# supersimple33/aruco-slam

Hardware: AMD Instinct MI355X
Metric: EKF updates/sec at n=1024 landmarks, m=32 obs/frame (higher is better)
Workload: dtype f32 covariance / f64 state

## Files before the change

aruco_slam_amd/csrc/ekf_api.hip:

```cpp
#include <atomic>
#include <cstring>

#include "ekf_host.h"
#include "ekf_kernels.h"

thread_local std::string g_err;

namespace {

std::atomic<ekf_filter*> g_pipelining{nullptr};

void release_pipelining_token(ekf_filter* f) { (void)g_pipelining.compare_exchange_strong(f, nullptr); }

constexpr int kStageSlots = 64;
constexpr int kMacroSuper = 8;
constexpr int kMacroMinTiles = 3000;
constexpr int kTimedKernels = 4;
constexpr int kWideVisible = 1024;
inline int visible_cap(int model) { return model == EKF_MODEL_ROTATIONS ? 50 : 64; }
inline bool wide_frame(int model, int m) { return m > visible_cap(model); }
constexpr int kEventPool = 2048;

struct Layout {
    int64_t cap;
// ... 197 lines not shown
    fr.jac = f->at<double>(L.off_jac);
    fr.resid = f->at<double>(L.off_resid);
    fr.lmcol = f->at<int32_t>(L.off_lmcol);
    fr.amat = f->at<double>(L.off_amat);
    fr.lda = L.cap;
    fr.sblk = f->at<double>(L.off_sblk);
    fr.sblk_rows = L.kmax;
    fr.lmat = f->at<double>(L.off_lmat);
    fr.ldl = L.kmax;
    fr.dinv = f->at<double>(L.off_dinv);
    fr.lop = f->at<double>(L.off_lop);
    fr.dop = f->at<double>(L.off_dop);
    fr.yvec = f->at<double>(L.off_y);
    fr.wpanel = f->at<void>(L.off_wpanel);
    fr.ldw = L.cap;
    fr.wdbg = f->debug_w ? f->at<double>(L.off_wdbg) : nullptr;
    fr.status = f->at<int32_t>(L.off_status);
    fr.traj_row = traj_row;
    fr.dxvec = f->at<double>(L.off_dx);
    fr.stamps = (f->debug_w || f->debug_stamps) ? f->at<long long>(L.off_stamps) : nullptr;
    fr.stamps_heavy = f->debug_stamps_light ? 0 : 1;
    fr.nz = EkfNoise{f->cfg.q_cam, f->cfg.q_err, f->cfg.q_lm, f->cfg.r_uncertainty};
    fr.quat_mode = f->cfg.quat_mode;
    fr.n_lm = f->n_lm;
    fr.state_host = nullptr;
    fr.status_host = nullptr;
    fr.cov_tiles = nullptr;
    fr.cov_grid = 0;
    if (f->tiles_T > 0 && f->tiles_T == (fr.dims + 127) / 128) {
        fr.cov_tiles = f->at<uint32_t>(L.off_tiles);
        fr.cov_grid = f->tiles_grid;
    }
    return fr;
}

bool use_front_kernel(const ekf_filter* f, const EkfFrame& fr) { return (f->cfg.flags & 4) == 0 && fr.kpad <= 192; }

void bind_exchange(ekf_filter* f, EkfFrame& fr) {
    const Layout& L = f->lay;
    double* base = f->at<double>(L.off_xl);
    fr.xl = base + (f->fseq & 1) * L.xl_len;
    fr.xl_next = base + ((f->fseq + 1) & 1) * L.xl_len;
    fr.xl_dop = (int32_t)L.xl_dop;
    fr.xl_y = (int32_t)L.xl_y;
    fr.xl_jac = (int32_t)L.xl_jac;
    fr.xl_tag = (int32_t)L.xl_tag;
    fr.xl_len = (int32_t)L.xl_len;
    fr.xs = fr.xl + L.xl_xs;
    fr.xr = fr.xl + L.xl_xr;
    fr.xs_tag = fr.xl + L.xl_stag;
    fr.seqno = (double)(f->fseq + 1);
    fr.done_ctr = f->at<unsigned long long>(L.off_done);
    f->done_total += (uint64_t)(fr.ncols / 64);
    fr.done_target = f->done_total;
    f->fseq++;
}

int ensure_tiles(ekf_filter* f) {
    const Layout& L = f->lay;
    const int T = (f->dims() + 127) / 128;
    const bool want = L.tiles_cap > 0 &&
                      (f->cfg.cov_kernel == EKF_COVK_MFMA_MACRO || T * (T + 1) / 2 >= kMacroMinTiles);
    if (!want) {
        f->tiles_T = -1;
        return EKF_OK;
    }
    if (f->tiles_T == T) return EKF_OK;
    HIP_TRY(hipStreamSynchronize(f->stream));
    HIP_TRY(hipStreamSynchronize(f->big));
    const int grid = ekf_cov_macro_table(T, kMacroSuper, f->tiles_host.at<uint32_t>(0), L.tiles_cap);
    if (grid <= 0) return fail(EKF_ERR_STATE, "macro-tile launch table does not fit the workspace");
    HIP_TRY(hipMemcpy(f->at<uint32_t>(L.off_tiles), f->tiles_host.get(), (size_t)grid * 4, hipMemcpyHostToDevice));
    f->tiles_T = T;
    f->tiles_grid = grid;
    return EKF_OK;
}

int enqueue_frame(ekf_filter* f, const int32_t* idx_dev, const double* z_dev, int m,
                  double* traj_row, bool mirror) {
    int trc = ensure_tiles(f);
    if (trc) return trc;
    EkfFrame fr = make_frame(f, idx_dev, z_dev, m, traj_row);
    const int variant = f->cfg.cov_kernel == EKF_COVK_VALU ? 1 : 2;
    hipEvent_t* ev = nullptr;
    if (f->timing) {
        if (f->ev_frames == kEventPool) {
            int rc = fold_timing(f);
            if (rc) return rc;
        }
        ev = &f->ev[f->ev_frames * (kTimedKernels + 1)];
        f->ev_frames++;
    }
    hipEvent_t* ev_all = (ev && !f->timing_cov_only) ? ev : nullptr;
    if (ev_all) HIP_TRY(hipEventRecord(ev[0], f->stream));
    const bool mirrored = use_front_kernel(f, fr) && !f->timing && mirror;
    if (use_front_kernel(f, fr)) {
        bind_exchange(f, fr);
        if (mirrored) {
            fr.state_host = f->readback.at<double>(256);
            fr.status_host = f->readback.at<int32_t>(128);
        }
        by_cov_type(f, [&](auto elem) { ekf_launch_front<decltype(elem)>(fr, f->stream); });
        if (ev_all) {
            HIP_TRY(hipEventRecord(ev[1], f->stream));
            HIP_TRY(hipEventRecord(ev[2], f->stream));
        }
    } else if (wide_frame(fr.model, m)) {
        const bool blocked = fr.kpad > EKF_WIDE_REUSE_ROWS;
        const int rp = blocked ? (int)round_up(fr.k, EKF_WIDE_BLOCK) : fr.kpad;
        double* aw = blocked ? f->at<double>(f->lay.off_wwork) : nullptr;
        if (blocked && !f->lay.off_wwork) return fail(EKF_ERR_STATE, "internal: no wide-frame workspace");
        by_cov_type(f, [&](auto elem) { ekf_launch_wide_front<decltype(elem)>(fr, aw, rp, f->stream); });
        if (ev_all) HIP_TRY(hipEventRecord(ev[1], f->stream));
        if (blocked) ekf_launch_wide_factor(fr, aw, f->at<double>(f->lay.off_xinv), rp, f->stream);
        else ekf_launch_solve(fr, f->stream);
        if (ev_all) HIP_TRY(hipEventRecord(ev[2], f->stream));
        by_cov_type(f, [&](auto elem) {
            if (blocked) ekf_launch_wide_finish<decltype(elem)>(fr, aw, f->stream);
            else ekf_launch_panel<decltype(elem)>(fr, f->stream);
        });
        if (fr.model == 1) ekf_launch_inject_rot(fr, f->n_lm, f->stream);
    } else {
        by_cov_type(f, [&](auto elem) { ekf_launch_gather<decltype(elem)>(fr, f->stream); });
        if (ev_all) HIP_TRY(hipEventRecord(ev[1], f->stream));
        ekf_launch_solve(fr, f->stream);
        if (ev_all) HIP_TRY(hipEventRecord(ev[2], f->stream));
        by_cov_type(f, [&](auto elem) { ekf_launch_panel<decltype(elem)>(fr, f->stream); });
        if (fr.model == 1) ekf_launch_inject_rot(fr, f->n_lm, f->stream);
    }
    f->shortcut.frame(!f->timing && hipEventRecord(f->ev_front, f->stream) == hipSuccess, mirrored);
    if (fr.kpad > EKF_WIDE_REUSE_ROWS) {
        if (ev) HIP_TRY(hipEventRecord(ev[3], f->stream));
        for (int r0 = 0; r0 < fr.kpad; r0 += EKF_WIDE_REUSE_ROWS) {
            EkfFrame cf = fr;
            cf.wpanel = static_cast<char*>(fr.wpanel) + (size_t)r0 * fr.ldw * f->lay.elem;
            cf.kpad = std::min(EKF_WIDE_REUSE_ROWS, fr.kpad - r0);
            cf.k = std::min(cf.kpad, std::max(0, fr.k - r0));
            if (r0 > 0) cf.nz.q_cam = cf.nz.q_err = cf.nz.q_lm = 0.0;
            by_cov_type(f, [&](auto elem) { ekf_launch_cov_update<decltype(elem)>(cf, variant, f->stream); });
        }
        if (ev) HIP_TRY(hipEventRecord(ev[4], f->stream));
    } else {
        by_cov_type(f, [&](auto elem) {
            ekf_launch_cov_update<decltype(elem)>(fr, variant, f->stream, ev ? ev[3] : nullptr, ev ? ev[4] : nullptr);
        });
    }
    HIP_TRY(hipGetLastError());
    f->last_m = m;
    return EKF_OK;
}

int check_ready(ekf_filter* f) {
    if (!f) return fail(EKF_ERR_INVALID, "filter handle is NULL");
    if (!f->bound) return fail(EKF_ERR_STATE, "ekf_bind_buffers has not been called");
    if (!f->is_reset) return fail(EKF_ERR_STATE, "ekf_reset has not been called");
    HIP_TRY(hipSetDevice(f->device));
    return EKF_OK;
}

int sync_and_check(ekf_filter* f, int state_count = 0) {
    if (state_count > 0 && f->shortcut.front_pending) {
        HIP_TRY(hipEventSynchronize(f->ev_front));
        if (f->shortcut.zero_copy() && *f->readback.at<volatile int32_t>(128) == 0)
            return EKF_OK;
        HIP_TRY(hipMemcpyAsync(f->readback.get(), f->at<int32_t>(f->lay.off_status), 32, hipMemcpyDeviceToHost, f->big));
        HIP_TRY(hipMemcpyAsync(f->readback.at<double>(256), f->state, (size_t)state_count * 8, hipMemcpyDeviceToHost, f->big));
        HIP_TRY(hipStreamSynchronize(f->big));
    } else {
        HIP_TRY(hipMemcpyAsync(f->readback.get(), f->at<int32_t>(f->lay.off_status), 32, hipMemcpyDeviceToHost, f->stream));
        if (state_count > 0)
            HIP_TRY(hipMemcpyAsync(f->readback.at<double>(256), f->state, (size_t)state_count * 8, hipMemcpyDeviceToHost, f->stream));
        HIP_TRY(hipStreamSynchronize(f->stream));
        release_pipelining_token(f);
    }
    const int32_t* info = f->readback.at<int32_t>(0);
    const int32_t st = info[0];
    f->shortcut.read_back(st == 0, state_count == f->dims());
    if (st != 0) {
        if (st & EKF_ST_BAD_INDEX)
            return fail(EKF_ERR_INVALID, "landmark index out of range in a device-resident detection array "
                                         "(clamped on the device; the filter state is no longer meaningful, reset it)");
        if (st & (EKF_ST_STALE_JAC | EKF_ST_STALE_COL | EKF_ST_STALE_S))
            return fail(EKF_ERR_NUMERIC, "internal: exchange data of another frame accepted in the front kernel (status " +
                                             std::to_string(st) + ")");
        if (st & EKF_ST_GATE_TIMEOUT)
            return fail(EKF_ERR_NUMERIC, "internal: a device-side wait between the two streams of the pipelined sequence mode timed out");
        if (st & EKF_ST_TIMEOUT)
            return fail(EKF_ERR_NUMERIC, "internal: exchange wait timed out in the front kernel (status " +
                                             std::to_string(st) + ")");
        if (info[2] >= 200)
            return fail(EKF_ERR_NUMERIC, "internal: a wait inside the factorisation workgroup timed out (flag word " +
                                             std::to_string(info[2] - 200) + ")");
        return fail(EKF_ERR_NUMERIC, "innovation covariance S was not positive definite (block column " +
                                         std::to_string(info[2] - 100) + ", wave mask " + std::to_string(info[1]) + ")");
    }
    return EKF_OK;
}

bool pipeline_wanted(const ekf_filter* f, int dims, int kpad, int m) {
    const bool auto_on = !(dims > 9000 && kpad > 96) && !(f->cfg.model == EKF_MODEL_ROTATIONS && kpad > 64);
    const bool want = (f->cfg.flags & 2) != 0 || ((f->cfg.flags & 1) == 0 && auto_on);
    return want && f->lay.has_cov2 && !f->timing && (f->cfg.flags & 4) == 0 && kpad <= 192 &&
           !wide_frame(f->cfg.model, m);
}

int probe_queues(ekf_filter* f) {
    if (f->la_ok >= 0) return EKF_OK;
    unsigned long long* probe = f->at<unsigned long long>(f->lay.off_sync) + 2;
    int32_t* pstat = f->at<int32_t>(f->lay.off_sync) + 8;
    f->la_ok = 0;
    for (int attempt = 0; attempt < 8 && f->la_ok == 0; ++attempt) {
        if (attempt > 0) {
            hipStream_t fresh = nullptr;
            HIP_TRY(hipStreamCreateWithFlags(&fresh, hipStreamNonBlocking));
            HIP_TRY(hipStreamSynchronize(f->big));
            (void)hipStreamDestroy(f->big);
            f->big = fresh;
        }
        HIP_TRY(hipMemsetAsync(probe, 0, 64, f->stream));
        HIP_TRY(hipStreamSynchronize(f->stream));
        ekf_launch_gate(probe, 1ull, pstat, f->big, 1 << 14);
        ekf_launch_signal(probe, 1ull, f->stream);
        HIP_TRY(hipStreamSynchronize(f->big));
        HIP_TRY(hipStreamSynchronize(f->stream));
        int32_t ps = 0;
        HIP_TRY(hipMemcpy(&ps, pstat, 4, hipMemcpyDeviceToHost));
        f->la_ok = (ps == 0) ? 1 : 0;
    }
    return EKF_OK;
}

bool take_pipelining_token(ekf_filter* f) {
    ekf_filter* owner = nullptr;
    if (!g_pipelining.compare_exchange_strong(owner, f) && owner != f) {
        bool idle = hipStreamQuery(owner->stream) == hipSuccess && hipStreamQuery(owner->big) == hipSuccess;
        (void)hipGetLastError();
        if (!(idle && g_pipelining.compare_exchange_strong(owner, f))) return false;
    }
    return true;
}

int choose_pipelining(ekf_filter* f, bool want_runs, int* mode) {
    *mode = EKF_SEQ_SERIAL;
    if (!want_runs) return EKF_OK;
    int rc = probe_queues(f);
    if (rc) return rc;
    if (f->la_ok == 0) *mode = EKF_SEQ_SERIAL_ONE_QUEUE;
    else if (!take_pipelining_token(f)) *mode = EKF_SEQ_SERIAL_OTHER_HANDLE;
    else *mode = EKF_SEQ_PIPELINED;
    return EKF_OK;
}

struct RunFrame {
    const int32_t* idx;
    const double* z;
    int m;
    double* traj_row;
};

template <class FrameAt>
int run_pipelined(ekf_filter* f, int frames, FrameAt frame_at, void* other) {
    const Layout& L = f->lay;
    int rc = ensure_tiles(f);
    if (rc) return rc;
    void* wbuf[2] = {f->at<void>(L.off_wpanel), f->at<void>(L.off_wpanel2)};
    void* cbuf[2] = {f->cov, other};
    char* wsup0 = f->at<char>(L.off_wsup);
    void* wsup[2] = {wsup0, wsup0 + (size_t)L.kmax * L.wsup_ld * L.elem};
    unsigned long long* sync = f->at<unsigned long long>(L.off_sync);
    int32_t* status = f->at<int32_t>(L.off_status);
    const uint64_t base = f->la_base;
    f->shortcut.run();
    RunFrame nx = frame_at(0);
    for (int t = 0; t < frames; ++t) {
        const int par = t & 1;
        const RunFrame cf_t = nx;
        EkfFrame fr = make_frame(f, cf_t.idx, cf_t.z, cf_t.m, cf_t.traj_row);
        fr.cov = cbuf[0];
        fr.wpanel = wbuf[par];
        if (t > 0) {
            fr.cov = cbuf[par ^ 1];
            fr.wprev = wbuf[par ^ 1];
            fr.wsup_prev = wsup[par ^ 1];
        }
        const int nb = fr.kpad / EKF_RB;
        const int grid = nb * (nb + 1) / 2 + 2 + fr.ncols / 64;
        fr.wsup_ld = L.wsup_ld;
        fr.la_sync = sync;
        fr.la_signal = (t > 0) ? base + (uint64_t)t : 0;
        fr.la_gate = (t > 0) ? base + (uint64_t)t : 0;
        fr.lds_min = grid <= 100 ? 148 * 1024 : 0;
        if (t + 1 < frames) {
            nx = frame_at(t + 1);
            fr.next_idx = nx.idx;
            fr.next_m = nx.m;
            fr.wsup = wsup[par];
        }
        bind_exchange(f, fr);
        by_cov_type(f, [&](auto elem) { ekf_launch_front<decltype(elem)>(fr, f->stream); });
        EkfFrame cu = fr;
        cu.cov = cbuf[par];
        cu.cov_out = cbuf[par ^ 1];
        if (t + 1 < frames) {
            ekf_launch_gate(sync, base + (uint64_t)t + 1, status, f->big);
            by_cov_type(f, [&](auto elem) { ekf_launch_cov_update<decltype(elem)>(cu, 2, f->big); });
            ekf_launch_signal(sync + 1, base + (uint64_t)t + 1, f->big);
        } else {
            by_cov_type(f, [&](auto elem) { ekf_launch_cov_update<decltype(elem)>(cu, 2, f->stream); });
        }
        HIP_TRY(hipGetLastError());
        f->last_m = cf_t.m;
    }
    f->cov = cbuf[frames & 1];
    f->la_base = base + (uint64_t)frames;
    return EKF_OK;
}

struct RunPlan {
    std::vector<char> candidate;
    std::vector<char> joins;
    bool want_runs = false;
};

template <class MOf, class NNewOf>
RunPlan plan_runs(const ekf_filter* f, int frames, MOf m_of, NNewOf nnew_of) {
    RunPlan p;
    p.candidate.assign((size_t)frames, 0);
    p.joins.assign((size_t)frames, 0);
    int prev_kpad = -1;
    int nn = f->n_lm;
    for (int t = 0; t < frames; ++t) {
        const int m = m_of(t);
        if (m == 0) continue;
        const int nnew = nnew_of(t);
        nn += nnew;
        const int kpad = (int)round_up(f->lay.rd * m, EKF_RB);
        p.candidate[t] = pipeline_wanted(f, f->lay.lmd * nn + EKF_CAM, kpad, m);
        p.joins[t] = p.candidate[t] && nnew == 0 && prev_kpad == kpad;
        p.want_runs = p.want_runs || p.joins[t];
        prev_kpad = p.candidate[t] ? kpad : -1;
    }
    return p;
}

template <class FrameOf, class FirstSightings>
int run_frames(ekf_filter* f, int frames, FrameOf frame_of, FirstSightings first_sightings, const RunPlan& plan, bool pipe_ok,
               int64_t* stats) {
    void* const home = f->cov;
    void* const spare = f->lay.has_cov2 ? f->at<void>(f->lay.off_cov2) : nullptr;
    std::vector<int> run;
    auto serial = [&](int t) {
        const RunFrame r = frame_of(t);
        if (stats) stats[0] += 1;
        return enqueue_frame(f, r.idx, r.z, r.m, r.traj_row, false);
    };
    auto flush = [&]() -> int {
        int rc = EKF_OK;
        if (run.size() == 1) {
            rc = serial(run[0]);
        } else if (run.size() >= 2) {
            rc = run_pipelined(f, (int)run.size(), [&](int i) { return frame_of(run[i]); }, f->cov == home ? spare : home);
            if (stats) {
                stats[0] += (int64_t)run.size();
                stats[1] += (int64_t)run.size();
                stats[2] += 1;
            }
        }
        run.clear();
        return rc;
    };
    int rc = EKF_OK;
    for (int t = 0; t < frames && rc == EKF_OK; ++t) {
        if (frame_of(t).m == 0) continue;
        const bool in_run = pipe_ok && plan.candidate[t];
        if (!(in_run && plan.joins[t])) {
            rc = flush();
            if (rc) break;
        }
        const int nnew = first_sightings(t);
        f->n_lm += nnew;
        if (stats) stats[3] += nnew;
        if (in_run) run.push_back(t);
        else rc = serial(t);
    }
    if (rc == EKF_OK) rc = flush();
    if (f->cov != home) {
        hipError_t e = hipMemcpyAsync(home, f->cov, (size_t)f->lay.cap * f->lay.cap * f->lay.elem, hipMemcpyDeviceToDevice,
                                      f->stream);
        f->cov = home;
        if (e != hipSuccess && rc == EKF_OK) rc = fail(EKF_ERR_HIP, std::string("hipMemcpyAsync: ") + hipGetErrorString(e));
    }
    return rc;
}

int reserve_host_buffers(ekf_filter* f, const Layout& L) {
    int rc = f->ring.reserve(L.slot_bytes * kStageSlots);
    if (rc == EKF_OK) rc = f->tiles_host.reserve((size_t)L.tiles_cap * 4);
    if (rc == EKF_OK) rc = f->readback.reserve(256 + (size_t)L.cap * 8);
    return rc;
}

int open_handle(ekf_filter* f) {
    int rc = reserve_host_buffers(f, f->lay);
    if (rc) return rc;
    HIP_TRY(hipStreamCreateWithFlags(&f->big, hipStreamNonBlocking));
    HIP_TRY(hipEventCreateWithFlags(&f->ev_front, hipEventDisableTiming));
    for (hipEvent_t& e : f->slot_done) HIP_TRY(hipEventCreateWithFlags(&e, hipEventDisableTiming));
    return EKF_OK;
}

int clear_buffers(const ekf_filter* f, void* cov, double* state, char* ws, const Layout& L) {
    HIP_TRY(hipMemsetAsync(cov, 0, (size_t)L.cap * L.cap * L.elem, f->stream));
    HIP_TRY(hipMemsetAsync(state, 0, (size_t)L.cap * 8, f->stream));
    HIP_TRY(hipMemsetAsync(ws, 0, L.total, f->stream));
    HIP_TRY(hipMemsetD32Async(reinterpret_cast<hipDeviceptr_t>(ws + L.off_xl), (int)0xFFFBADC0u, L.xl_len * 4, f->stream));
    return EKF_OK;
}

void restart_workspace(ekf_filter* f) {
    f->fseq = 0;
    f->done_total = 0;
    f->la_base = 0;
    f->tiles_T = -1;
    std::memset(f->readback.get(), 0, 256 + (size_t)f->lay.cap * 8);
}

}

extern "C" {

const char* ekf_last_error_string(void) { return g_err.c_str(); }

int ekf_default_config(ekf_config* cfg) {
    if (!cfg) return fail(EKF_ERR_INVALID, "config is NULL");
    std::memset(cfg, 0, sizeof(*cfg));
    cfg->max_landmarks = 50;
    cfg->max_visible = 50;
    cfg->cov_dtype = EKF_COV_F64;
    cfg->quat_mode = EKF_QUAT_AS_WRITTEN;
    cfg->cov_kernel = EKF_COVK_AUTO;
    cfg->model = EKF_MODEL_EKF;
    cfg->initial_camera_uncertainty = 0.1;
    cfg->initial_landmark_uncertainty = 0.7;
    cfg->r_uncertainty = 0.9;
    cfg->q_cam = 0.3;
    cfg->q_err = 0.5;
    cfg->q_lm = 0.01;
    cfg->stream = nullptr;
    return EKF_OK;
}

int ekf_query_sizes(const ekf_config* cfg, int64_t* ld, size_t* cov_bytes, size_t* state_bytes,
                    size_t* workspace_bytes) {
    int rc = check_config(cfg);
    if (rc) return rc;
    Layout L = make_layout(*cfg);
    if (ld) *ld = L.cap;
    if (cov_bytes) *cov_bytes = (size_t)L.cap * L.cap * L.elem;
    if (state_bytes) *state_bytes = (size_t)L.cap * 8;
    if (workspace_bytes) *workspace_bytes = L.total;
    return EKF_OK;
}

int ekf_create(const ekf_config* cfg, ekf_filter** out) {
    int rc = check_config(cfg);
    if (rc) return rc;
    if (!out) return fail(EKF_ERR_INVALID, "out is NULL");
    int ndev = 0;
    HIP_TRY(hipGetDeviceCount(&ndev));
    if (ndev < 1) return fail(EKF_ERR_HIP, "no HIP device visible");
    ekf_filter* f = new ekf_filter();
    if (hipGetDevice(&f->device) != hipSuccess) f->device = 0;
    f->cfg = *cfg;
    f->lay = make_layout(*cfg);
    f->stream = static_cast<hipStream_t>(cfg->stream);
    rc = open_handle(f);
    if (rc) {
        ekf_destroy(f);
        return rc;
    }
    *out = f;
    return EKF_OK;
}

int ekf_destroy(ekf_filter* f) {
    if (!f) return EKF_OK;
    (void)hipStreamSynchronize(f->stream);
    if (f->big) {
        (void)hipStreamSynchronize(f->big);
        (void)hipStreamDestroy(f->big);
    }
    release_pipelining_token(f);
    if (f->ev_front) (void)hipEventDestroy(f->ev_front);
    for (auto& e : f->ev) (void)hipEventDestroy(e);
    for (int i = 0; i < kStageSlots; ++i)
        if (f->slot_done[i]) (void)hipEventDestroy(f->slot_done[i]);
    for (auto& e : f->log_pin_done)
        if (e) (void)hipEventDestroy(e);
    delete f;
    return EKF_OK;
}

int ekf_bind_buffers(ekf_filter* f, void* cov_dev, int64_t ld, double* state_dev, void* workspace_dev,
                     size_t workspace_bytes) {
    if (!f) return fail(EKF_ERR_INVALID, "filter handle is NULL");
    int rc = check_device_buffers({cov_dev, state_dev, workspace_dev}, workspace_bytes, f->lay.total, "ekf_query_sizes");
    if (rc) return rc;
    if (ld != f->lay.cap) return fail(EKF_ERR_INVALID, "ld must equal the value from ekf_query_sizes");
    f->cov = cov_dev;
    f->ld = ld;
    f->state = state_dev;
    f->ws = static_cast<char*>(workspace_dev);
    f->bound = true;
    f->is_reset = false;
    f->tiles_T = -1;
    return EKF_OK;
}

int ekf_grow(ekf_filter* f, int32_t new_max_landmarks, int32_t new_max_visible, void* cov_dev, int64_t ld, double* state_dev,
             void* workspace_dev, size_t workspace_bytes) {
    if (!f) return fail(EKF_ERR_INVALID, "filter handle is NULL");
    if (!f->bound || !f->is_reset) return fail(EKF_ERR_STATE, "ekf_grow needs a bound, reset filter");
    if (new_max_landmarks < f->cfg.max_landmarks || new_max_visible < f->cfg.max_visible)
        return fail(EKF_ERR_INVALID, "ekf_grow cannot shrink the capacity");
    ekf_config ncfg = f->cfg;
    ncfg.max_landmarks = new_max_landmarks;
    ncfg.max_visible = new_max_visible;
    int rc = check_config(&ncfg);
    if (rc) return rc;
    const Layout nl = make_layout(ncfg);
    rc = check_device_buffers({cov_dev, state_dev, workspace_dev}, workspace_bytes, nl.total,
                              "ekf_query_sizes for the new capacity");
    if (rc) return rc;
    if (ld != nl.cap) return fail(EKF_ERR_INVALID, "ld must equal the value from ekf_query_sizes for the new capacity");
    if (cov_dev == f->cov || state_dev == f->state || workspace_dev == static_cast<void*>(f->ws))
        return fail(EKF_ERR_INVALID, "ekf_grow needs NEW buffers (the old ones are read)");
    HIP_TRY(hipSetDevice(f->device));
    HIP_TRY(hipStreamSynchronize(f->stream));
    HIP_TRY(hipStreamSynchronize(f->big));
    release_pipelining_token(f);
    const Layout& ol = f->lay;
    char* nws = static_cast<char*>(workspace_dev);
    rc = clear_buffers(f, cov_dev, state_dev, nws, nl);
    if (rc) return rc;
    HIP_TRY(hipMemcpyAsync(state_dev, f->state, (size_t)ol.cap * 8, hipMemcpyDeviceToDevice, f->stream));
    HIP_TRY(hipMemcpy2DAsync(cov_dev, (size_t)nl.cap * nl.elem, f->cov, (size_t)ol.cap * ol.elem, (size_t)ol.cap * ol.elem,
                             (size_t)ol.cap, hipMemcpyDeviceToDevice, f->stream));
    HIP_TRY(hipMemcpyAsync(nws + nl.off_status, f->ws + ol.off_status, 32, hipMemcpyDeviceToDevice, f->stream));
    HIP_TRY(hipStreamSynchronize(f->stream));
    rc = reserve_host_buffers(f, nl);
    if (rc) return rc;
    f->cfg = ncfg;
    f->lay = nl;
    f->cov = cov_dev;
    f->ld = ld;
    f->state = state_dev;
    f->ws = nws;
    restart_workspace(f);
    f->shortcut.new_workspace();
    return EKF_OK;
}

int ekf_reset(ekf_filter* f, const double initial_camera_pose[10]) {
    if (!f) return fail(EKF_ERR_INVALID, "filter handle is NULL");
    if (!f->bound) return fail(EKF_ERR_STATE, "ekf_bind_buffers has not been called");
    if (!initial_camera_pose) return fail(EKF_ERR_INVALID, "initial pose is NULL");
    HIP_TRY(hipSetDevice(f->device));
    const Layout& L = f->lay;
    HIP_TRY(hipStreamSynchronize(f->stream));
    int rc = clear_buffers(f, f->cov, f->state, f->ws, L);
    if (rc) return rc;
    restart_workspace(f);
    f->shortcut.reset();
    HIP_TRY(hipMemcpyAsync(f->state, initial_camera_pose, 10 * sizeof(double), hipMemcpyHostToDevice,
                           f->stream));
    char diag[8 * EKF_CAM];
    by_cov_type(f, [&](auto elem) {
        for (int i = 0; i < EKF_CAM; ++i)
            reinterpret_cast<decltype(elem)*>(diag)[i] = (decltype(elem))f->cfg.initial_camera_uncertainty;
    });
    HIP_TRY(hipMemcpy2DAsync(f->cov, (size_t)(L.cap + 1) * L.elem, diag, L.elem, L.elem, EKF_CAM,
                             hipMemcpyHostToDevice, f->stream));
    HIP_TRY(hipStreamSynchronize(f->stream));
    f->n_lm = 0;
    f->last_m = 0;
    f->is_reset = true;
    return EKF_OK;
}

int ekf_add_markers(ekf_filter* f, const double* cam_frame_xyz, const double* diag_uncertainty,
                    int32_t count) {
    int rc = check_ready(f);
    if (rc) return rc;
    if (count < 0 || (count > 0 && !cam_frame_xyz)) return fail(EKF_ERR_INVALID, "bad marker list");
    if (f->n_lm + count > f->cfg.max_landmarks)
        return fail(EKF_ERR_CAPACITY, "more landmarks than max_landmarks");
    const Layout& L = f->lay;
    f->shortcut.markers_added();
    int done = 0;
    while (done < count) {
        const int chunk = std::min(256, count - done);
        char* slot = f->ring.get() + (size_t)f->slot * L.slot_bytes;
        HIP_TRY(hipEventSynchronize(f->slot_done[f->slot]));
        double* hx = reinterpret_cast<double*>(slot);
        double* hu = reinterpret_cast<double*>(slot + align256(256 * 48));
        const bool rot = f->cfg.model == EKF_MODEL_ROTATIONS;
// ... 442 lines not shown
```

aruco_slam_amd/csrc/ekf_cov_update.hip:

```cpp
#include <hip/hip_ext.h>
#include "ekf_kernels.h"

template <typename T>
__device__ __forceinline__ void ekf_cov_store(T* p, T v) {
    __hip_atomic_store(p, v, __ATOMIC_RELAXED, __HIP_MEMORY_SCOPE_AGENT);
}

typedef float f32x16 __attribute__((ext_vector_type(16)));
typedef double f64x4 __attribute__((ext_vector_type(4)));

template <typename T>
__global__ __launch_bounds__(256) void ekf_cov_update_valu(EkfFrame fr) {
    __shared__ T sa[16][64];
    __shared__ T sb[16][64];
    const int tid = threadIdx.x, tx = tid & 15, ty = tid >> 4;
    const int i0 = blockIdx.y * 64, j0 = blockIdx.x * 64;
    const T* __restrict__ wp = static_cast<const T*>(fr.wpanel);
    T acc[4][4];
#pragma unroll
    for (int x = 0; x < 4; ++x)
#pragma unroll
        for (int y = 0; y < 4; ++y) acc[x][y] = (T)0;
    for (int kc = 0; kc < fr.kpad; kc += 16) {
#pragma unroll
        for (int t = 0; t < 4; ++t) {
            const int e = tid + 256 * t, r = e >> 6, cc = e & 63;
            sa[r][cc] = wp[(int64_t)(kc + r) * fr.ldw + i0 + cc];
            sb[r][cc] = wp[(int64_t)(kc + r) * fr.ldw + j0 + cc];
        }
        __syncthreads();
#pragma unroll
        for (int r = 0; r < 16; ++r) {
            T a[4], b[4];
#pragma unroll
            for (int x = 0; x < 4; ++x) a[x] = -sa[r][ty * 4 + x];
#pragma unroll
            for (int y = 0; y < 4; ++y) b[y] = sb[r][tx * 4 + y];
#pragma unroll
            for (int x = 0; x < 4; ++x)
#pragma unroll
                for (int y = 0; y < 4; ++y) acc[x][y] = __builtin_fma(a[x], b[y], acc[x][y]);
        }
        __syncthreads();
    }
    T* __restrict__ P = static_cast<T*>(fr.cov);
#pragma unroll
    for (int x = 0; x < 4; ++x) {
        const int row = i0 + ty * 4 + x;
#pragma unroll
        for (int y = 0; y < 4; ++y) {
            const int col = j0 + tx * 4 + y;
            T v = P[(int64_t)row * fr.ld + col];
            if (row == col) v += (T)ekf_qdiag(row, fr.dims, fr.nz);
            P[(int64_t)row * fr.ld + col] = v + acc[x][y];
        }
    }
}

__device__ __forceinline__ void ekf_tri_decode(int item, int& I, int& J) {
    int i = (int)((sqrtf(8.0f * (float)item + 1.0f) - 1.0f) * 0.5f);
    while (i * (i + 1) / 2 > item) --i;
    while ((i + 1) * (i + 2) / 2 <= item) ++i;
    I = i;
    J = item - i * (i + 1) / 2;
}

template <int KB, int DMAX = 3, int WPE = 5>
__global__ __launch_bounds__(256) __attribute__((amdgpu_waves_per_eu(WPE, WPE)))
void ekf_cov_update_mfma_f32(EkfFrame fr, int nitems) {
    __shared__ float tr[4][32][33];
    const int wave = threadIdx.x >> 6, lane = threadIdx.x & 63;
    const int l31 = lane & 31, lhi = lane >> 5;
    const int item = __builtin_amdgcn_readfirstlane(blockIdx.x * 4 + wave);
    if (item >= nitems) return;
    int I, J;
    ekf_tri_decode(item, I, J);
    const int i0 = 32 * I, j0 = 32 * J;
    const float* __restrict__ wp = static_cast<const float*>(fr.wpanel);
    const float* __restrict__ P = static_cast<const float*>(fr.cov);
    float* Pout = fr.cov_out ? static_cast<float*>(fr.cov_out) : static_cast<float*>(fr.cov);
    const int ld = (int)fr.ld, ldw = (int)fr.ldw;
    constexpr int NCH = KB, D = (NCH < DMAX) ? NCH : DMAX;
    float ra[D][8], rb[D][8], pt[16];
    const unsigned wlane = 4u * (unsigned)(lhi * ldw + l31);
    const unsigned plane = 4u * (unsigned)(4 * lhi * ld + l31);
    const uint64_t kstep = 8ull * (uint64_t)ldw;
    uint64_t ua = reinterpret_cast<uint64_t>(wp + i0), ub = reinterpret_cast<uint64_t>(wp + j0);
    const float* __restrict__ ptile = P + (int64_t)i0 * ld + j0;
    float* otile = Pout + (int64_t)i0 * ld + j0;
#define EKF_GLD(dst, voff, sbase) asm volatile("global_load_dword %0, %1, %2" : "=v"(dst) : "v"(voff), "s"(sbase) : "memory")
#define EKF_WAIT16(n, A, B)                                                                              \
    asm volatile("s_waitcnt vmcnt(%16)"                                                                   \
                 : "+v"(A[0]), "+v"(A[1]), "+v"(A[2]), "+v"(A[3]), "+v"(A[4]), "+v"(A[5]), "+v"(A[6]), "+v"(A[7]), \
                   "+v"(B[0]), "+v"(B[1]), "+v"(B[2]), "+v"(B[3]), "+v"(B[4]), "+v"(B[5]), "+v"(B[6]), "+v"(B[7])  \
                 : "n"(n))
    f32x16 acc;
#pragma unroll
    for (int r = 0; r < 16; ++r) acc[r] = 0.0f;
#pragma unroll
    for (int c = 0; c < D; ++c) {
#pragma unroll
        for (int u = 0; u < 8; ++u) {
            EKF_GLD(ra[c][u], wlane, ua);
            EKF_GLD(rb[c][u], wlane, ub);
            ua += kstep;
            ub += kstep;
        }
    }
    {
        uint64_t pb = reinterpret_cast<uint64_t>(ptile);
        const uint64_t r1 = 4ull * (uint64_t)ld, r5 = 20ull * (uint64_t)ld;
#pragma unroll
        for (int reg = 0; reg < 16; ++reg) {
            EKF_GLD(pt[reg], plane, pb);
            pb += ((reg & 3) == 3) ? r5 : r1;
        }
    }
#pragma unroll
    for (int c = 0; c < NCH; ++c) {
        const int later = (c < NCH - D) ? c : NCH - D;
        const int allow = (c < D) ? 16 * (D - c - 1) + 16 + 16 * later : 16 * (D + later - c - 1);
        switch (allow) {
            case 0: EKF_WAIT16(0, ra[c % D], rb[c % D]); break;
            case 16: EKF_WAIT16(16, ra[c % D], rb[c % D]); break;
            case 32: EKF_WAIT16(32, ra[c % D], rb[c % D]); break;
            case 48: EKF_WAIT16(48, ra[c % D], rb[c % D]); break;
            default: EKF_WAIT16(63, ra[c % D], rb[c % D]); break;
        }
#pragma unroll
        for (int u = 0; u < 8; ++u)
            acc = __builtin_amdgcn_mfma_f32_32x32x2f32(-ra[c % D][u], rb[c % D][u], acc, 0, 0, 0);
        __builtin_amdgcn_sched_barrier(0);
        if (c + D < NCH) {
#pragma unroll
            for (int u = 0; u < 8; ++u) {
                EKF_GLD(ra[c % D][u], wlane, ua);
                EKF_GLD(rb[c % D][u], wlane, ub);
                ua += kstep;
                ub += kstep;
            }
        }
        __builtin_amdgcn_sched_barrier(0);
    }
    asm volatile("s_waitcnt vmcnt(0)"
                 : "+v"(pt[0]), "+v"(pt[1]), "+v"(pt[2]), "+v"(pt[3]), "+v"(pt[4]), "+v"(pt[5]), "+v"(pt[6]), "+v"(pt[7]),
                   "+v"(pt[8]), "+v"(pt[9]), "+v"(pt[10]), "+v"(pt[11]), "+v"(pt[12]), "+v"(pt[13]), "+v"(pt[14]), "+v"(pt[15]));
#undef EKF_GLD
#undef EKF_WAIT16
    const float qlane = (I == J) ? (float)ekf_qdiag(i0 + l31, fr.dims, fr.nz) : 0.0f;
    float out[16];
    auto stf = [](float* base, unsigned off, float v) { ekf_cov_store(reinterpret_cast<float*>(reinterpret_cast<char*>(base) + off), v); };
#pragma unroll
    for (int reg = 0; reg < 16; ++reg) {
        const int rl = (reg & 3) + 8 * (reg >> 2) + 4 * lhi;
        const float v = (pt[reg] + ((rl == l31) ? qlane : 0.0f)) + acc[reg];
        out[reg] = v;
        stf(otile + (int64_t)((reg & 3) + 8 * (reg >> 2)) * ld, plane, v);
    }
    if (I != J) {
#pragma unroll
        for (int reg = 0; reg < 16; ++reg)
            tr[wave][(reg & 3) + 8 * (reg >> 2) + 4 * lhi][l31] = out[reg];
        __builtin_amdgcn_wave_barrier();
        float* pm = Pout + (int64_t)j0 * ld + i0;
        const unsigned mlane = 4u * (unsigned)(lhi * ld + l31);
#pragma unroll
        for (int it = 0; it < 16; ++it)
            stf(pm + (int64_t)(2 * it) * ld, mlane, tr[wave][l31][2 * it + lhi]);
    }
}

__global__ __launch_bounds__(256) void ekf_cov_update_mfma_f64(EkfFrame fr, int nitems) {
    __shared__ double tr[4][32][33];
    const int wave = threadIdx.x >> 6, lane = threadIdx.x & 63;
    const int c = lane & 15, g = lane >> 4;
    const int item = blockIdx.x * 4 + wave;
    if (item >= nitems) return;
    int I, J;
    ekf_tri_decode(item, I, J);
    const int i0 = 32 * I, j0 = 32 * J;
    const double* __restrict__ wp = static_cast<const double*>(fr.wpanel);
    const double* P = static_cast<const double*>(fr.cov);
    double* Pout = fr.cov_out ? static_cast<double*>(fr.cov_out) : static_cast<double*>(fr.cov);
    const int64_t ld = fr.ld, ldw = fr.ldw;

    double pt[2][2][4];
#pragma unroll
    for (int ri = 0; ri < 2; ++ri)
#pragma unroll
        for (int ci = 0; ci < 2; ++ci)
#pragma unroll
            for (int r = 0; r < 4; ++r)
                pt[ri][ci][r] = P[(int64_t)(i0 + 16 * ri + g + 4 * r) * ld + j0 + 16 * ci + c];
    f64x4 acc[2][2];
#pragma unroll
    for (int ri = 0; ri < 2; ++ri)
#pragma unroll
        for (int ci = 0; ci < 2; ++ci)
#pragma unroll
            for (int r = 0; r < 4; ++r) acc[ri][ci][r] = 0.0;
    const double* wa = wp + (int64_t)g * ldw + i0 + c;
    const double* wb = wp + (int64_t)g * ldw + j0 + c;
    const int steps = fr.kpad >> 2;
    for (int ks = 0; ks < steps; ks += 4) {
        double a0[4], a1[4], b0[4], b1[4];
#pragma unroll
        for (int u = 0; u < 4; ++u) {
            const int64_t off = (int64_t)(4 * (ks + u)) * ldw;
            a0[u] = wa[off];
            a1[u] = wa[off + 16];
            b0[u] = wb[off];
            b1[u] = wb[off + 16];
        }
#pragma unroll
        for (int u = 0; u < 4; ++u) {
            acc[0][0] = __builtin_amdgcn_mfma_f64_16x16x4f64(-a0[u], b0[u], acc[0][0], 0, 0, 0);
            acc[0][1] = __builtin_amdgcn_mfma_f64_16x16x4f64(-a0[u], b1[u], acc[0][1], 0, 0, 0);
            acc[1][0] = __builtin_amdgcn_mfma_f64_16x16x4f64(-a1[u], b0[u], acc[1][0], 0, 0, 0);
            acc[1][1] = __builtin_amdgcn_mfma_f64_16x16x4f64(-a1[u], b1[u], acc[1][1], 0, 0, 0);
        }
    }
#pragma unroll
    for (int ri = 0; ri < 2; ++ri)
#pragma unroll
        for (int ci = 0; ci < 2; ++ci)
#pragma unroll
            for (int r = 0; r < 4; ++r) {
                const int rl = 16 * ri + g + 4 * r, cl = 16 * ci + c;
                double v = pt[ri][ci][r];
                if (I == J && rl == cl) v += ekf_qdiag(i0 + rl, fr.dims, fr.nz);
                v += acc[ri][ci][r];
                ekf_cov_store(Pout + (int64_t)(i0 + rl) * ld + j0 + cl, v);
                if (I != J) tr[wave][rl][cl] = v;
            }
    if (I != J) {
        __builtin_amdgcn_wave_barrier();
        const int l31 = lane & 31, lhi = lane >> 5;
#pragma unroll
        for (int it = 0; it < 16; ++it) {
            const int cc = 2 * it + lhi;
            ekf_cov_store(Pout + (int64_t)(j0 + cc) * ld + i0 + l31, tr[wave][l31][cc]);
        }
    }
}

__global__ __launch_bounds__(256) void ekf_cov_update_mfma_f64_split(EkfFrame fr, int nitems) {
    __shared__ double tr[32][33];
    const int wave = threadIdx.x >> 6, lane = threadIdx.x & 63;
    const int c = lane & 15, g = lane >> 4;
    const int ri = wave >> 1, ci = wave & 1;
    int I, J;
    ekf_tri_decode(blockIdx.x, I, J);
    const int i0 = 32 * I, j0 = 32 * J;
    const double* __restrict__ wp = static_cast<const double*>(fr.wpanel);
    const double* P = static_cast<const double*>(fr.cov);
    double* Pout = fr.cov_out ? static_cast<double*>(fr.cov_out) : static_cast<double*>(fr.cov);
    const int64_t ld = fr.ld, ldw = fr.ldw;
    double pt[4];
#pragma unroll
    for (int r = 0; r < 4; ++r) pt[r] = P[(int64_t)(i0 + 16 * ri + g + 4 * r) * ld + j0 + 16 * ci + c];
    f64x4 acc = {0.0, 0.0, 0.0, 0.0};
    const double* wa = wp + (int64_t)g * ldw + i0 + 16 * ri + c;
    const double* wb = wp + (int64_t)g * ldw + j0 + 16 * ci + c;
    const int steps = fr.kpad >> 2;
    for (int ks = 0; ks < steps; ks += 4) {
        double a[4], b[4];
#pragma unroll
        for (int u = 0; u < 4; ++u) {
            const int64_t off = (int64_t)(4 * (ks + u)) * ldw;
            a[u] = wa[off];
            b[u] = wb[off];
        }
#pragma unroll
        for (int u = 0; u < 4; ++u) acc = __builtin_amdgcn_mfma_f64_16x16x4f64(-a[u], b[u], acc, 0, 0, 0);
    }
#pragma unroll
    for (int r = 0; r < 4; ++r) {
        const int rl = 16 * ri + g + 4 * r, cl = 16 * ci + c;
        double v = pt[r];
        if (I == J && rl == cl) v += ekf_qdiag(i0 + rl, fr.dims, fr.nz);
        v += acc[r];
        ekf_cov_store(Pout + (int64_t)(i0 + rl) * ld + j0 + cl, v);
        if (I != J) tr[rl][cl] = v;
    }
    if (I != J) {
        __syncthreads();
        const int l31 = threadIdx.x & 31;
        for (int cc = threadIdx.x >> 5; cc < 32; cc += 8)
            ekf_cov_store(Pout + (int64_t)(j0 + cc) * ld + i0 + l31, tr[l31][cc]);
    }
}

__global__ void ekf_gate_kernel(unsigned long long* counter, unsigned long long target, int32_t* status, int max_polls) {
    if (threadIdx.x != 0) return;
    int it = 0;
    while (__hip_atomic_load(counter, __ATOMIC_RELAXED, __HIP_MEMORY_SCOPE_SYSTEM) < target) {
        if (++it > max_polls) { atomicOr(status, EKF_ST_GATE_TIMEOUT); break; }
        __builtin_amdgcn_s_sleep(8);
    }
}
__global__ void ekf_signal_kernel(unsigned long long* counter, unsigned long long value) {
    if (threadIdx.x == 0) __hip_atomic_store(counter, value, __ATOMIC_RELAXED, __HIP_MEMORY_SCOPE_SYSTEM);
}
void ekf_launch_gate(unsigned long long* counter, unsigned long long target, int32_t* status, hipStream_t s, int max_polls) {
    hipLaunchKernelGGL(ekf_gate_kernel, dim3(1), dim3(64), 0, s, counter, target, status, max_polls);
}
void ekf_launch_signal(unsigned long long* counter, unsigned long long value, hipStream_t s) {
    hipLaunchKernelGGL(ekf_signal_kernel, dim3(1), dim3(64), 0, s, counter, value);
}

#define EKF_COV_LAUNCH(kernel, grid, block, s, e0, e1, ...)                                     \
    do {                                                                                         \
        if (e0) hipExtLaunchKernelGGL(kernel, grid, block, 0, s, e0, e1, 0, __VA_ARGS__);        \
        else hipLaunchKernelGGL(kernel, grid, block, 0, s, __VA_ARGS__);                         \
    } while (0)

static inline int ekf_tri_items(const EkfFrame& fr) {
    const int t = (fr.dims + 31) / 32;
    return t * (t + 1) / 2;
}

template <>
void ekf_launch_cov_update<float>(const EkfFrame& fr, int variant, hipStream_t s, hipEvent_t e0, hipEvent_t e1) {
    if (variant == 1) {
        EKF_COV_LAUNCH(ekf_cov_update_valu<float>, dim3(fr.ncols / 64, fr.ncols / 64), dim3(256), s, e0, e1, fr);
    } else if (fr.cov_tiles) {
        ekf_launch_cov_update_macro(fr, s, e0, e1);
    } else {
        const int items = ekf_tri_items(fr);
        const dim3 grid((items + 3) / 4), block(256);
        switch (fr.kpad / 16) {
#define EKF_COV_CASE(KB) case KB: EKF_COV_LAUNCH((ekf_cov_update_mfma_f32<KB, 3, (KB <= 8) ? 5 : 4>), grid, block, s, e0, e1, fr, items); break;
            EKF_COV_CASE(1) EKF_COV_CASE(2) EKF_COV_CASE(3) EKF_COV_CASE(4) EKF_COV_CASE(5) EKF_COV_CASE(6)
            EKF_COV_CASE(7) EKF_COV_CASE(8) EKF_COV_CASE(9) EKF_COV_CASE(10) EKF_COV_CASE(11) EKF_COV_CASE(12)
            EKF_COV_CASE(13) EKF_COV_CASE(14) EKF_COV_CASE(15) EKF_COV_CASE(16) EKF_COV_CASE(17) EKF_COV_CASE(18)
            EKF_COV_CASE(19) EKF_COV_CASE(20) EKF_COV_CASE(21) EKF_COV_CASE(22) EKF_COV_CASE(23) EKF_COV_CASE(24)
            default: break;
#undef EKF_COV_CASE
        }
    }
}
template <>
void ekf_launch_cov_update<double>(const EkfFrame& fr, int variant, hipStream_t s, hipEvent_t e0, hipEvent_t e1) {
    if (variant == 1) {
        EKF_COV_LAUNCH(ekf_cov_update_valu<double>, dim3(fr.ncols / 64, fr.ncols / 64), dim3(256), s, e0, e1, fr);
    } else {
        const int items = ekf_tri_items(fr);
        if (items <= 2048)
            EKF_COV_LAUNCH(ekf_cov_update_mfma_f64_split, dim3(items), dim3(256), s, e0, e1, fr, items);
        else
            EKF_COV_LAUNCH(ekf_cov_update_mfma_f64, dim3((items + 3) / 4), dim3(256), s, e0, e1, fr, items);
    }
}
```

aruco_slam_amd/csrc/ekf_kernels.h:

```cpp
#pragma once
#include <hip/hip_runtime.h>
#include <stdint.h>
#include "ekf_device.h"

#define EKF_ST_NOT_SPD 1
#define EKF_ST_TIMEOUT 4
#define EKF_ST_STALE_JAC 16
#define EKF_ST_STALE_COL 32
#define EKF_ST_STALE_S 64
#define EKF_ST_BAD_INDEX 128
#define EKF_ST_GATE_TIMEOUT 256

struct EkfFrame {
    void* cov;
    int64_t ld;
    double* state;
    int32_t model;
    int32_t dims;
    int32_t ncols;
    int32_t m;
    int32_t k;
    int32_t kpad;
    const int32_t* idx;
    const double* z;
    double* jac;
    double* resid;
    int32_t* lmcol;
    double* amat;
    int64_t lda;
    double* sblk;
    int32_t sblk_rows;
    double* lmat;
    int32_t ldl;
    double* dinv;
    double* lop;
    double* dop;
    double* yvec;
    void* wpanel;
    int64_t ldw;
    double* wdbg;
    int32_t* status;
    double* traj_row;
    double* dxvec;
    long long* stamps;
    int32_t stamps_heavy;
    const int32_t* next_idx;
    int32_t next_m;
    void* cov_out;
    const void* wprev;
    const void* wsup_prev;
    unsigned long long* la_sync;
    unsigned long long la_signal, la_gate;
    int32_t lds_min;
    void* wsup;
    int32_t wsup_ld;
    EkfNoise nz;
    int32_t quat_mode;
    double* xl;
    double* xl_next;
    int32_t xl_dop, xl_y, xl_jac;
    int32_t xl_len;
    double* xs;
    double* xr;
    double* xs_tag;
    int32_t n_lm;
    unsigned long long* done_ctr;
    unsigned long long done_target;
    int32_t xl_tag;
    double seqno;
    double* state_host;
    int32_t* status_host;
    const uint32_t* cov_tiles;
    int32_t cov_grid;
};

__device__ __forceinline__ void ekf_raise(const EkfFrame& fr, int bits) {
    atomicOr(fr.status, bits);
    if (fr.status_host) __hip_atomic_store(fr.status_host, 1, __ATOMIC_RELAXED, __HIP_MEMORY_SCOPE_SYSTEM);
}

__device__ __forceinline__ int ekf_lm_column(const EkfFrame& fr, int lmd, int j, bool flag) {
    int i = fr.idx[j];
    if ((unsigned)i >= (unsigned)fr.n_lm) {
        if (flag) ekf_raise(fr, EKF_ST_BAD_INDEX);
        i = 0;
    }
    return EKF_CAM + lmd * i;
}

__device__ inline void ekf_inject_camera(const EkfFrame& fr, const double err[3], const double x[3]) {
    double q[4] = {fr.state[3], fr.state[4], fr.state[5], fr.state[6]};
    ekf_quat_inject(q, err, fr.quat_mode);
    for (int i = 0; i < 4; ++i) fr.state[3 + i] = q[i];
    for (int i = 0; i < 3; ++i) fr.state[7 + i] = 0.0;
    if (fr.traj_row) {
        fr.traj_row[0] = x[0]; fr.traj_row[1] = x[1]; fr.traj_row[2] = x[2];
        for (int i = 0; i < 4; ++i) fr.traj_row[3 + i] = q[i];
    }
}

template <typename T> void ekf_launch_front(const EkfFrame& fr, hipStream_t s);
template <typename T> void ekf_launch_gather(const EkfFrame& fr, hipStream_t s);
void ekf_launch_solve(const EkfFrame& fr, hipStream_t s);
template <typename T> void ekf_launch_panel(const EkfFrame& fr, hipStream_t s);
template <typename T> void ekf_launch_cov_update(const EkfFrame& fr, int variant, hipStream_t s,
                                                 hipEvent_t e0 = nullptr, hipEvent_t e1 = nullptr);
void ekf_launch_cov_update_macro(const EkfFrame& fr, hipStream_t s, hipEvent_t e0 = nullptr, hipEvent_t e1 = nullptr);
int ekf_cov_macro_table(int T, int S, uint32_t* out, int capacity);
void ekf_launch_gate(unsigned long long* counter, unsigned long long target, int32_t* status, hipStream_t s,
                     int max_polls = 1 << 22);
void ekf_launch_signal(unsigned long long* counter, unsigned long long value, hipStream_t s);

#define EKF_WIDE_REUSE_ROWS 384
#define EKF_WIDE_BLOCK 64
template <typename T> void ekf_launch_wide_front(const EkfFrame& fr, double* aw, int rp, hipStream_t s);
void ekf_launch_wide_factor(const EkfFrame& fr, double* aw, double* xinv, int rp, hipStream_t s);
template <typename T> void ekf_launch_wide_finish(const EkfFrame& fr, const double* aw, hipStream_t s);

template <typename T>
void ekf_launch_add_markers(void* cov, int64_t ld, double* state, int32_t dims,
                            const double* xyz_dev, const double* unc_dev, double default_unc,
                            int32_t count, hipStream_t s);
void ekf_launch_inject_rot(const EkfFrame& fr, int n_lm, hipStream_t s);
template <typename T>
void ekf_launch_add_markers_rot(void* cov, int64_t ld, double* state, int32_t dims, const double* pose6_dev,
                                const double* unc_dev, double default_unc, int32_t count, hipStream_t s);
void ekf_launch_log_prepare(const double* poses_dev, int64_t count, int rd, double* z_dev, hipStream_t s);
template <typename T>
void ekf_launch_log_add_markers(int model, void* cov, int64_t ld, double* state, int32_t dims, const double* poses_dev,
                                const int32_t* slots_dev, double default_unc, int32_t count, hipStream_t s);
void ekf_launch_log_fill_rows(double* traj_dev, const int32_t* pairs, int32_t count, const double* state, hipStream_t s);
template <typename T>
void ekf_launch_cov_diag(const void* cov, int64_t ld, double* out_dev, int32_t count, hipStream_t s);

#define EKF_BATCH_MAX_LANDMARKS 82
#define EKF_BATCH_MAX_VISIBLE 16
#define EKF_BATCH_ROT_MAX_LANDMARKS 24
#define EKF_BATCH_ROT_MAX_VISIBLE 8
#define EKF_BATCH_ST_NUMERIC (-5)
struct EkfBatchWindow {
    double* P;
    int64_t ld;
    double* state;
    const double* noise;
    int32_t* status;
    int32_t* nlm;
    const int32_t* lm_index;
    const int64_t* frame_offsets;
    const int64_t* member_frames;
    const double* poses;
    double* traj;
    double* nis;
    double* cam_cov;
    int32_t quat_mode;
    int32_t window_first, window_frames;
    int32_t kmax, lda;
};
extern "C" size_t ekf_batch_lds_bytes(int kmax, int lda);
extern "C" size_t ekf_batch_rot_lds_bytes(int kmax, int lda);
void ekf_launch_batch_window(const EkfBatchWindow& a, int members, hipStream_t s);
void ekf_launch_batch_rot_window(const EkfBatchWindow& a, int members, hipStream_t s);
#define EKF_BATCH_LARGE_MAX_LANDMARKS 338
#define EKF_BATCH_ROT_LARGE_MAX_LANDMARKS 101
struct EkfBatchLargeWindow {
    EkfBatchWindow w;
    double* W;
    int64_t w_stride;
};
extern "C" size_t ekf_batch_large_lds_bytes(int model, int kmax);
void ekf_launch_batch_large_window(int model, const EkfBatchLargeWindow& g, int members, hipStream_t s);
#define EKF_BATCH_WIDE_MAX_VISIBLE 64
#define EKF_BATCH_ROT_WIDE_MAX_VISIBLE 50
extern "C" size_t ekf_batch_wide_lds_bytes(int model, int kmax);
void ekf_launch_batch_wide_window(int model, const EkfBatchLargeWindow& g, int members, hipStream_t s);
#define EKF_REPLICA_CHUNK 64
void ekf_launch_replica_poses(const double* poses_dev, int64_t D, const double* sigma, int32_t count, uint64_t seed,
                              uint32_t r0, double* out_dev, hipStream_t s);

struct EkfCamera {
    double fx, fy, cx, cy;
    double k[8];
};
void ekf_launch_ippe_square(const double* corners_dev, int count, double marker_size, const EkfCamera& cam,
                            double* poses_dev, hipStream_t s);
```

Before: 42540.

## Write only lower-triangle covariance tiles plus mirrored rows needed by next-next frame

In the pipelined multi-frame path, the covariance update kernel now stores only the lower-triangle tiles. It skips the full transpose mirror of off-diagonal tiles into the upper triangle, and instead mirrors only the rows belonging to the camera block and the landmarks observed two frames ahead, which the front stage will read. The aim is to cut global store traffic and LDS transposes in the bandwidth-bound symmetric update. The risk is correctness: any consumer reading upper-triangle entries outside the marked rows would see stale data, and the new path depends on the mark indices being correct.

```diff
diff --git a/aruco_slam_amd/csrc/ekf_api.hip b/aruco_slam_amd/csrc/ekf_api.hip
--- a/aruco_slam_amd/csrc/ekf_api.hip
+++ b/aruco_slam_amd/csrc/ekf_api.hip
@@ -523,6 +523,12 @@
         cu.cov = cbuf[par];
         cu.cov_out = cbuf[par ^ 1];
         if (t + 1 < frames) {
+            cu.cov_lower = 1;
+            if (t + 2 < frames) {
+                const RunFrame f2 = frame_at(t + 2);
+                cu.mark_idx = f2.idx;
+                cu.mark_m = f2.m;
+            }
             ekf_launch_gate(sync, base + (uint64_t)t + 1, status, f->big);
             by_cov_type(f, [&](auto elem) { ekf_launch_cov_update<decltype(elem)>(cu, 2, f->big); });
             ekf_launch_signal(sync + 1, base + (uint64_t)t + 1, f->big);
diff --git a/aruco_slam_amd/csrc/ekf_cov_update.hip b/aruco_slam_amd/csrc/ekf_cov_update.hip
--- a/aruco_slam_amd/csrc/ekf_cov_update.hip
+++ b/aruco_slam_amd/csrc/ekf_cov_update.hip
@@ -65,7 +65,7 @@
     J = item - i * (i + 1) / 2;
 }
 
-template <int KB, int DMAX = 3, int WPE = 5>
+template <int KB, int DMAX = 3, int WPE = 5, bool LOWER = false>
 __global__ __launch_bounds__(256) __attribute__((amdgpu_waves_per_eu(WPE, WPE)))
 void ekf_cov_update_mfma_f32(EkfFrame fr, int nitems) {
     __shared__ float tr[4][32][33];
@@ -73,6 +73,10 @@
     const int l31 = lane & 31, lhi = lane >> 5;
     const int item = __builtin_amdgcn_readfirstlane(blockIdx.x * 4 + wave);
     if (item >= nitems) return;
+    int mk = 0;
+    if constexpr (LOWER) {
+        if (lane < fr.mark_m) mk = fr.mark_idx[lane];
+    }
     int I, J;
     ekf_tri_decode(item, I, J);
     const int i0 = 32 * I, j0 = 32 * J;
@@ -157,7 +161,28 @@
         out[reg] = v;
         stf(otile + (int64_t)((reg & 3) + 8 * (reg >> 2)) * ld, plane, v);
     }
-    if (I != J) {
+    if constexpr (LOWER) {
+        if (I == J) return;
+        asm volatile("" : "+v"(mk));
+        const int lmd = (fr.model == 1) ? EkfModel<1>::LMD : EkfModel<0>::LMD;
+        unsigned bits = (j0 == 0 && fr.mark_m > 0) ? (1u << EKF_CAM) - 1u : 0u;
+        if (lane < fr.mark_m) {
+            const int li = ((unsigned)mk >= (unsigned)fr.n_lm) ? 0 : mk;
+            const int lo = EKF_CAM + lmd * li - j0;
+            const uint64_t run = (1ull << lmd) - 1ull;
+            if (lo > -lmd && lo < 32) bits |= (unsigned)(lo >= 0 ? run << lo : run >> -lo);
+        }
+#pragma unroll
+        for (int sh = 32; sh > 0; sh >>= 1) bits |= (unsigned)__shfl_xor((int)bits, sh);
+        const unsigned mark = __builtin_amdgcn_readfirstlane(bits);
+        if (mark != 0u && ((mark >> l31) & 1u)) {
+            typedef float f32x4 __attribute__((ext_vector_type(4)));
+            float* pr = Pout + (int64_t)(j0 + l31) * ld + i0 + 4 * lhi;
+#pragma unroll
+            for (int q = 0; q < 4; ++q)
+                *reinterpret_cast<f32x4*>(pr + 8 * q) = f32x4{out[4 * q], out[4 * q + 1], out[4 * q + 2], out[4 * q + 3]};
+        }
+    } else if (I != J) {
 #pragma unroll
         for (int reg = 0; reg < 16; ++reg)
             tr[wave][(reg & 3) + 8 * (reg >> 2) + 4 * lhi][l31] = out[reg];
@@ -326,6 +351,17 @@
         EKF_COV_LAUNCH(ekf_cov_update_valu<float>, dim3(fr.ncols / 64, fr.ncols / 64), dim3(256), s, e0, e1, fr);
     } else if (fr.cov_tiles) {
         ekf_launch_cov_update_macro(fr, s, e0, e1);
+    } else if (fr.cov_lower && fr.mark_m <= 64 && fr.kpad <= 192) {
+        const int items = ekf_tri_items(fr);
+        const dim3 grid((items + 3) / 4), block(256);
+        switch (fr.kpad / 16) {
+#define EKF_COV_LOWER_CASE(KB) case KB: EKF_COV_LAUNCH((ekf_cov_update_mfma_f32<KB, 3, (KB <= 8) ? 5 : 4, true>), grid, block, s, e0, e1, fr, items); break;
+            EKF_COV_LOWER_CASE(1) EKF_COV_LOWER_CASE(2) EKF_COV_LOWER_CASE(3) EKF_COV_LOWER_CASE(4) EKF_COV_LOWER_CASE(5)
+            EKF_COV_LOWER_CASE(6) EKF_COV_LOWER_CASE(7) EKF_COV_LOWER_CASE(8) EKF_COV_LOWER_CASE(9) EKF_COV_LOWER_CASE(10)
+            EKF_COV_LOWER_CASE(11) EKF_COV_LOWER_CASE(12)
+            default: break;
+#undef EKF_COV_LOWER_CASE
+        }
     } else {
         const int items = ekf_tri_items(fr);
         const dim3 grid((items + 3) / 4), block(256);
diff --git a/aruco_slam_amd/csrc/ekf_kernels.h b/aruco_slam_amd/csrc/ekf_kernels.h
--- a/aruco_slam_amd/csrc/ekf_kernels.h
+++ b/aruco_slam_amd/csrc/ekf_kernels.h
@@ -47,6 +47,9 @@
     const int32_t* next_idx;
     int32_t next_m;
     void* cov_out;
+    int32_t cov_lower;
+    const int32_t* mark_idx;
+    int32_t mark_m;
     const void* wprev;
     const void* wsup_prev;
     unsigned long long* la_sync;
```

New measurement: 42850 (median of 6 runs). About the same (+0.7%).
